# SergioAlvarezB/calibration-normalizing-flows

Measured on AMD Instinct MI355X. Metric: logit-vectors/sec forward+log-det (6-layer RealNVP, D=10), higher is better.
Workload: dtype f32; 1 GPU; cfg2: 6-layer RealNVP coupling, D=10, hidden_size=[5, 5], 1048576 vectors per GPU; global_batch=1048576, parallelism=dp1, weights=N(0,0.1) synthetic

## Files before the change

calibration-normalizing-flows_amd/csrc/cnf_sgpr.hip:

```cpp
#include <hip/hip_runtime.h>

#include <mutex>
#include <type_traits>
#include <unordered_map>

#include "cnf_internal.h"
#include "cnf_valu_common.h"
#include "cnf_valu_io.h"
#include "cnf_sgpr_common.h"

#ifdef CNF_SGPR_TRACE
__device__ unsigned long long cnf_trace[16384 * 8];
__device__ unsigned long long cnf_trace_clk[16384 * 2];
#define CNF_TRC(slot)                                                                   \
  do {                                                                                  \
    if (lane == 0 && gw < 16384) cnf_trace_clk[gw * 2 + (slot)] = __builtin_amdgcn_s_memtime(); \
  } while (0)
#define CNF_TR(slot)                                                                   \
  do {                                                                                 \
    if (lane == 0 && gw < 16384) cnf_trace[gw * 8 + (slot)] = __builtin_amdgcn_s_memrealtime(); \
  } while (0)
#else
#define CNF_TR(slot) \
  do {               \
  } while (0)
#define CNF_TRC(slot) \
  do {                \
  } while (0)
#endif

namespace cnf {
namespace {

using namespace valu;

constexpr int kWaves = 4;

template <bool ALL, bool PERM>
constexpr int pairs_per_lane() { return 1; }
template <int MODE, bool ALL, bool PERM>
constexpr int waves_per_simd() { return PERM ? 4 : 6; }

enum Mode { kFwd = 0, kInv = 1, kLoss = 2, kPredict = 3 };



template <int D, int H1, int H2, int P>
struct Act {
  f2 c[P][D - D / 2];
  f2 h1[P][H1 > 0 ? H1 : 1];
  f2 h2[P][H2 > 0 ? H2 : 1];
  f2 t[P][D / 2];
};

template <int NIN, int NOUT, int S, bool RELU, int P, int NC, class X, class E, class F>
__device__ __forceinline__ void slin(const SW<NC>& w, X&& x, E&& emit, F&& before) {
  sready();
  before();
  f2 a[NOUT][P];
#pragma unroll
  for (int o = 0; o < NOUT; ++o)
#pragma unroll
    for (int q = 0; q < P; ++q) {
      if constexpr (RELU && NIN == 1) a[o][q] = fma_wb_clamp(w.pair(o * S), x(q, 0));
      else a[o][q] = fma_wb(w.pair(o * S), x(q, 0));
    }
#pragma unroll
  for (int k = 1; k < NIN; ++k)
#pragma unroll
    for (int o = 0; o < NOUT; ++o)
#pragma unroll
      for (int q = 0; q < P; ++q) {
        if (RELU && k == NIN - 1) a[o][q] = fma_ws_clamp(w, o * S + 1 + k, x(q, k), a[o][q]);
        else a[o][q] = fma_ws(w, o * S + 1 + k, x(q, k), a[o][q]);
      }
#pragma unroll
  for (int o = 0; o < NOUT; ++o) emit(o, a[o]);
}

template <class S, int NETS, int IDX>
__device__ __forceinline__ constexpr int lin_at() {
  return ((NETS == 2 && IDX < S::NL) ? S::NF : 0) + S::off(IDX % S::NL);
}

template <class S, int NETS, int P, int IDX, int PAR, bool NEXT, class AC, class U>
__device__ __forceinline__ void run_seq(AC& ac, SW<S::NC>& A, SW<S::NC>& Bf, const float* wl,
                                        const float* wn, U&& upd) {
  constexpr int NL = S::NL, N = NETS * NL;
  if constexpr (IDX < N) {
    constexpr int i = IDX % NL;
    constexpr bool tnet = IDX < NL, last = i == NL - 1;
    constexpr bool odd = ((IDX + PAR) & 1) != 0;
    SW<S::NC>& cur = odd ? Bf : A;
    SW<S::NC>& nxt = odd ? A : Bf;
    auto x = [&](int q, int k) -> f2 {
      if constexpr (i == 0) return ac.c[q][k];
      else if constexpr (i == 1) return ac.h1[q][k];
      else return ac.h2[q][k];
    };
    auto emit = [&](int o, const f2* a) {
#pragma unroll
      for (int q = 0; q < P; ++q) {
        if constexpr (!last) {
          if constexpr (i == 0) ac.h1[q][o] = a[q];
          else ac.h2[q][o] = a[q];
        } else if constexpr (tnet && NETS == 2) {
          ac.t[q][o] = a[q];
        }
      }
      if constexpr (last && (!tnet || NETS == 1)) upd(o, a);
    };
    slin<S::nin(i), S::nout(i), S::stride(i), !last, P>(cur, x, emit, [&]() {
      if constexpr (IDX + 1 < N)
        sissue(nxt, wl + lin_at<S, NETS, IDX + 1>());
      else if constexpr (NEXT)
        sissue(nxt, wn + lin_at<S, NETS, 0>());
    });
    run_seq<S, NETS, P, IDX + 1, PAR, NEXT>(ac, A, Bf, wl, wn, upd);
  }
}

template <int D, int H1, int H2, bool INV, bool O, int NETS, bool PERM, bool NEXT, int P>
__device__ __forceinline__ void sp_step(f2 (&v)[P][D], f2 (&ld)[P], SW<SP<D, H1, H2>::NC>& A,
                                        SW<SP<D, H1, H2>::NC>& Bf, const float* wl,
                                        const float* wn, bool perm,
                                        const int32_t* __restrict__ q) {
  using S = SP<D, H1, H2>;
  constexpr int DT = S::DT, DC = S::DC;
  constexpr bool OC = INV ? !O : O;
  if constexpr (INV && PERM) {
    if (perm) {
#pragma unroll
      for (int p = 0; p < P; ++p) permute<D, O>(v[p], q);
    }
  }
  Act<D, H1, H2, P> ac;
#pragma unroll
  for (int p = 0; p < P; ++p)
#pragma unroll
    for (int k = 0; k < DC; ++k) ac.c[p][k] = v[p][R<D, OC>(DT + k)];
  auto upd = [&](int j, const f2* a) {
#pragma unroll
    for (int p = 0; p < P; ++p) {
      f2& x = v[p][R<D, OC>(j)];
      if constexpr (NETS == 1) {
        x = INV ? x - a[p] : x + a[p];
      } else if constexpr (!INV) {
        x = fmaV(x, exp2T(a[p]), ac.t[p][j]);
        ld[p] += a[p];
      } else {
        x = (x - ac.t[p][j]) * exp2T(-a[p]);
        ld[p] -= a[p];
      }
    }
  };
  run_seq<S, NETS, P, 0, O ? (NETS * S::NL) & 1 : 0, NEXT>(ac, A, Bf, wl, wn, upd);
  if constexpr (!INV && PERM) {
    if (perm) {
#pragma unroll
      for (int p = 0; p < P; ++p) permute<D, O>(v[p], q);
    }
  }
}

__device__ __forceinline__ float max3f(float a, float b, float c) {
  float r;
  asm("v_max3_f32 %0, %1, %2, %3" : "=v"(r) : "v"(a), "v"(b), "v"(c));
  return r;
}
__device__ __forceinline__ float max2f(float a, float b) {
  float r;
  asm("v_max_f32 %0, %1, %2" : "=v"(r) : "v"(a), "v"(b));
  return r;
}
template <int D>
__device__ __forceinline__ f2 pair_max(const f2* v) {
  f2 m;
#pragma unroll
  for (int q = 0; q < 2; ++q) {
    float r = v[0][q];
    int j = 1;
#pragma unroll
    for (; j + 1 < D; j += 2) r = max3f(r, v[j][q], v[j + 1][q]);
    if (j < D) r = max2f(r, v[j][q]);
    m[q] = r;
  }
  return m;
}

template <int D, int GATHER>
__device__ __forceinline__ void pair_loss(const f2* v, f2 ld, uint32_t lab2, int rows, int kind,
                                          float det, float& t0, float& t1, float& t2,
                                          const float* tile) {
  const uint32_t b0 = lab2 & 0xffu, b1 = (lab2 >> 8) & 0xffu;
  const bool ok[2] = {b0 != 0xffu, b1 != 0xffu};
  constexpr float kL2E = 1.4426950408889634f, kLN2 = 0.6931471805599453f;
  float zy[2];
  if constexpr (GATHER == 1) {
    zy[0] = tile[ok[0] ? (int)b0 : 0];
    zy[1] = tile[D + (ok[1] ? (int)b1 : 0)];
  }
  const f2 m = pair_max<D>(v);
  const f2 nm = m * splat(-kL2E, f2{});
  f2 se = exp2T(fmaT(kL2E, v[0], nm));
#pragma unroll
  for (int j = 1; j < D; ++j) se += exp2T(fmaT(kL2E, v[j], nm));
  if constexpr (GATHER == 0) {
    uint32_t za[D], zb[D];
#pragma unroll
    for (int j = 0; j < D; ++j) {
      za[j] = __float_as_uint(v[j].x);
      zb[j] = __float_as_uint(v[j].y);
    }
    zy[0] = __uint_as_float(sel_tree<D>(za, ok[0] ? (int)b0 : 0, 0));
    zy[1] = __uint_as_float(sel_tree<D>(zb, ok[1] ? (int)b1 : 0, 0));
  }
#pragma unroll
  for (int q = 0; q < 2; ++q) {
    if (q >= rows) continue;
    const float lpy = zy[q] - (m[q] + __builtin_amdgcn_logf(se[q]) * kLN2);
    const float l = ld[q];
    float ce, loss;
    if (kind == CNF_LOSS_CAL) {
      ce = -__builtin_amdgcn_logf(__builtin_amdgcn_exp2f(lpy * kL2E) + 1e-7f) * kLN2;
      loss = ce - l;
    } else {
      ce = -lpy;
      loss = ce - det * l;
    }
    if (!ok[q]) ce = loss = __builtin_nanf("");
    t0 += loss;
    t1 += ce;
    t2 += l;
  }
}

template <int D, bool O>
__device__ __forceinline__ void centre(f2* v) {
  f2 s = v[R<D, O>(0)];
#pragma unroll
  for (int j = 1; j < D; ++j) s += v[R<D, O>(j)];
  const f2 mu = s * splat(1.f / D, f2{});
#pragma unroll
  for (int j = 0; j < D; ++j) v[j] -= mu;
}

template <int D>
__device__ __forceinline__ void pair_predict(f2* v, const float* __restrict__ lp) {
  constexpr float kL2E = 1.4426950408889634f, kLN2 = 0.6931471805599453f;
  const f2 m = pair_max<D>(v);
  const f2 nm = m * splat(-kL2E, f2{});
  f2 e[D], se = splat(0.f, f2{});
#pragma unroll
  for (int j = 0; j < D; ++j) {
    e[j] = exp2T(fmaT(kL2E, v[j], nm));
    se += e[j];
  }
  const f2 inv = f2{1.f / se.x, 1.f / se.y};
  f2 a[D];
#pragma unroll
  for (int j = 0; j < D; ++j) {
    const f2 p = e[j] * inv + splat(1e-7f, f2{});
    a[j] = f2{__builtin_amdgcn_logf(p.x), __builtin_amdgcn_logf(p.y)} * splat(kLN2, f2{}) -
           splat(lp[j], f2{});
  }
  const f2 m2 = pair_max<D>(a);
  const f2 nm2 = m2 * splat(-kL2E, f2{});
  f2 s2 = splat(0.f, f2{});
#pragma unroll
  for (int j = 0; j < D; ++j) {
    a[j] = exp2T(fmaT(kL2E, a[j], nm2));
    s2 += a[j];
  }
  const f2 inv2 = f2{1.f / s2.x, 1.f / s2.y};
#pragma unroll
  for (int j = 0; j < D; ++j) v[j] = a[j] * inv2;
}

struct KArgs {
  float* out;
  float* ld;
  float* all;
  const int64_t* y;
  float* part;
  const void *reserved0, *reserved1, *reserved2;
  int L, kind;
  float det;
};

template <int D, int H1, int H2, int NETS, int MODE, bool ALL, bool PERM>
__global__ __launch_bounds__(kWaves * 64, (waves_per_simd<MODE, ALL, PERM>())) void k_sgpr(
    const float* __restrict__ in,
    int64_t B,
    const float* __restrict__ W,
    const int32_t* __restrict__ qtab,
    const int32_t* __restrict__ lflag,
    const float* __restrict__ lpri,
    KArgs a) {
  using S = SP<D, H1, H2>;
  constexpr int P = pairs_per_lane<ALL, PERM>();
  constexpr bool INV = MODE == kInv;
  constexpr int LF = NETS * S::NF;
  constexpr int TR = 128 * P;
  constexpr int TF = TR * D;
  extern __shared__ __attribute__((aligned(16))) float smem[];
  const int lane = threadIdx.x & 63;
  const int wv = __builtin_amdgcn_readfirstlane(threadIdx.x >> 6);
  float* sm = smem + wv * TF;
  const int L = a.L;
  const int nfull = (int)(B / TR), ntiles = (int)((B + TR - 1) / TR);
  const int gw = blockIdx.x * kWaves + wv, nw = gridDim.x * kWaves;
  int left = gw < ntiles ? (ntiles - 1 - gw) / nw + 1 : 0;
  auto layer_of = [&](int i) { return INV ? L - 1 - i : i; };
  auto align_of = [](const void* q) {
    const int m = (int)(reinterpret_cast<uintptr_t>(q) & 15);
    return m == 0 ? 16 : ((m & 7) == 0 ? 8 : 4);
  };
  [[maybe_unused]] const int al = a.out ? align_of(a.out) : 16;
  const int al_ld = a.ld ? align_of(a.ld) : 16;
  const bool y16 = MODE == kLoss && (reinterpret_cast<uintptr_t>(a.y) & 15) == 0;
  float lp[MODE == kPredict ? D : 1];
  if constexpr (MODE == kPredict) {
#pragma unroll
    for (int j = 0; j < D; ++j) lp[j] = lpri[j];
  }
  float lt0 = 0.f, lt1 = 0.f, lt2 = 0.f;

  const bool odd = (L & 1) != 0;
  auto compute = [&](f2 (&v)[P][D], f2 (&ld)[P], int64_t row0, int nr) {
#pragma unroll
    for (int p = 0; p < P; ++p) {
      if constexpr (MODE == kPredict) {
        if (odd) centre<D, true>(v[p]);
        else centre<D, false>(v[p]);
      }
      ld[p] = splat(0.f, f2{});
    }
    auto st_all = [&](int i, auto O_) {
      if constexpr (ALL) {
        constexpr bool O = decltype(O_)::value;
        f2 o[P][D];
#pragma unroll
        for (int p = 0; p < P; ++p)
#pragma unroll
          for (int j = 0; j < D; ++j) o[p][j] = v[p][R<D, O>(j)];
        store_rows<D, P>(a.all + ((int64_t)i * B + row0 + 2 * P * lane) * D, o, nr, 16);
      }
    };
    int i = 0;
    if (odd) {
      const int la = layer_of(0);
      const bool pa = PERM && (lflag[la] & kFlagPerm);
      const float* wa = W + (int64_t)la * LF;
      SW<S::NC> cur, alt;
      if constexpr (((NETS * S::NL) & 1) != 0) sissue(alt, wa + lin_at<S, NETS, 0>());
      else sissue(cur, wa + lin_at<S, NETS, 0>());
      sp_step<D, H1, H2, INV, true, NETS, PERM, false, P>(v, ld, cur, alt, wa, nullptr, pa,
                                                          qtab + la * D);
      st_all(0, std::false_type{});
      i = 1;
    }
    for (; i + 1 < L; i += 2) {
      const int la = layer_of(i), lb = layer_of(i + 1);
      const bool pa = PERM && (lflag[la] & kFlagPerm);
      const bool pb = PERM && (lflag[lb] & kFlagPerm);
      const float* wa = W + (int64_t)la * LF;
      const float* wb = W + (int64_t)lb * LF;
      SW<S::NC> cur, alt;
      sissue(cur, wa + lin_at<S, NETS, 0>());
      sp_step<D, H1, H2, INV, false, NETS, PERM, true, P>(v, ld, cur, alt, wa, wb, pa,
                                                          qtab + la * D);
      st_all(i, std::true_type{});
      sp_step<D, H1, H2, INV, true, NETS, PERM, false, P>(v, ld, cur, alt, wb, nullptr, pb,
                                                          qtab + lb * D);
      st_all(i + 1, std::false_type{});
    }
#pragma unroll
    for (int p = 0; p < P; ++p) {
      if constexpr (NETS == 2) ld[p] = ld[p] * splat(0.69314718055994531f, f2{});
      if constexpr (MODE == kPredict) pair_predict<D>(v[p], lp);
    }
  };
  auto loss = [&](const f2 (&v)[P][D], const f2 (&ld)[P], uint32_t lab, int nr,
                  const float* tile, auto gather) {
#pragma unroll
    for (int p = 0; p < P; ++p) {
      const int r = nr - 2 * p;
      constexpr int G = decltype(gather)::value;
      pair_loss<D, G>(v[p], ld[p], lab >> (16 * p), r < 0 ? 0 : (r > 2 ? 2 : r), a.kind, a.det,
                      lt0, lt1, lt2, tile + 2 * D * p);
    }
  };

  CNF_TR(0);
  CNF_TRC(0);
#ifdef CNF_SGPR_TRACE
  if (lane == 0 && gw < 16384)
    cnf_trace[gw * 8 + 7] = ((unsigned long long)__builtin_amdgcn_s_getreg((31 << 11) | 20) << 32) |
                            __builtin_amdgcn_s_getreg((31 << 11) | 4);
  int ntr = 0;
#endif
  int t = gw;
  if (t < nfull) wave_dma<D, TR>(sm, in + (int64_t)t * TF, lane);
  auto set_prio = [&]() {
    --left;
    if (left >= 3) __builtin_amdgcn_s_setprio(3);
    else if (left == 2) __builtin_amdgcn_s_setprio(2);
    else if (left == 1) __builtin_amdgcn_s_setprio(1);
    else __builtin_amdgcn_s_setprio(0);
  };
  for (; t < nfull; t += nw) {
    set_prio();
    asm volatile("s_waitcnt vmcnt(0)" ::: "memory");
    f2 v[P][D];
    if constexpr (P == 1) {
      if (odd) read_pairs_wait<D, true>(sm, lane, v);
      else read_pairs_wait<D, false>(sm, lane, v);
    } else {
      if (odd) read_pairs<D, P, true>(sm, lane, v);
      else read_pairs<D, P, false>(sm, lane, v);
      asm volatile("s_waitcnt lgkmcnt(0)" ::: "memory");
    }
#ifdef CNF_SGPR_TRACE
    if (ntr < 2) CNF_TR(1 + 2 * ntr);
#endif
    const int64_t row0 = (int64_t)t * TR;
    uint32_t lab = 0;
    if constexpr (MODE == kLoss) lab = load_labels<D, P>(a.y + row0 + 2 * P * lane, 2 * P, y16);
    f2 ld[P];
    compute(v, ld, row0, 2 * P);
    if constexpr (MODE == kLoss) {
      stage_pairs<D, P>(sm, lane, v);
      loss(v, ld, lab, 2 * P, sm + 2 * P * D * lane, std::integral_constant<int, 1>{});
    }
#ifdef CNF_SGPR_TRACE
    if (ntr < 2) CNF_TR(2 + 2 * ntr);
    CNF_TR(5);
    ++ntr;
#endif
    if (a.out) {
      if (MODE != kLoss) stage_pairs<D, P>(sm, lane, v);
      store_tile<TF>(a.out + row0 * D, sm, lane);
    }
    if (a.ld) store_lds<P>(a.ld + row0 + 2 * P * lane, ld, 2 * P, al_ld);
    asm volatile("s_waitcnt lgkmcnt(0)" ::: "memory");
    if (t + nw < nfull) wave_dma<D, TR>(sm, in + (int64_t)(t + nw) * TF, lane);
  }
  if (t == nfull && nfull < ntiles) {
    const int64_t row0 = (int64_t)t * TR;
    const int64_t r = row0 + 2 * P * lane;
    const int64_t left_rows = B - r;
    const int nr = left_rows <= 0 ? 0 : (left_rows >= 2 * P ? 2 * P : (int)left_rows);
    f2 v[P][D];
    auto load_rows = [&](auto O_) {
      constexpr bool O = decltype(O_)::value;
#pragma unroll
      for (int p = 0; p < P; ++p)
#pragma unroll
        for (int k = 0; k < D; ++k) {
          v[p][R<D, O>(k)].x = 2 * p < nr ? in[(r + 2 * p) * D + k] : 0.f;
          v[p][R<D, O>(k)].y = 2 * p + 1 < nr ? in[(r + 2 * p + 1) * D + k] : 0.f;
        }
    };
    if (odd) load_rows(std::true_type{});
    else load_rows(std::false_type{});
    uint32_t lab = 0;
    if constexpr (MODE == kLoss) lab = load_labels<D, P>(a.y + r, nr, false);
    f2 ld[P];
    compute(v, ld, row0, nr);
    if constexpr (MODE == kLoss) loss(v, ld, lab, nr, sm, std::integral_constant<int, 0>{});
    if (a.out) store_rows<D, P>(a.out + r * D, v, nr, 4);
    if (a.ld) store_lds<P>(a.ld + r, ld, nr, 4);
  }
  CNF_TRC(1);
  CNF_TR(6);
  if constexpr (MODE == kLoss) block_sum3<kWaves * 64>(lt0, lt1, lt2, smem, a.part);
}

using KFn = void (*)(const float*, int64_t, const float*, const int32_t*, const int32_t*,
                     const float*, KArgs);

struct KV {
  KFn fn;
  int tr;
};

enum Var { vFwd, vInv, vLoss, vPredict, kNVar };

struct SEntry {
  int D, H1, H2;
  KV fn[2][kNVar];
  KV pfn[2][3];
};

#define CNF_K(D, H1, H2, N, M, A, P) \
  {k_sgpr<D, H1, H2, N, M, A, P>, 128 * pairs_per_lane<A, P>()}
#define CNF_SV(D, H1, H2, N)                                                                  \
  {CNF_K(D, H1, H2, N, kFwd, false, false), CNF_K(D, H1, H2, N, kInv, false, false),           \
   CNF_K(D, H1, H2, N, kLoss, false, false), CNF_K(D, H1, H2, N, kPredict, false, false)}
#define CNF_SP(D, H1, H2, N)                                                                  \
  {CNF_K(D, H1, H2, N, kFwd, false, true), CNF_K(D, H1, H2, N, kInv, false, true),             \
   CNF_K(D, H1, H2, N, kPredict, false, true)}
#define CNF_SGPR(D, H1, H2) \
  {D, H1, H2, {CNF_SV(D, H1, H2, 1), CNF_SV(D, H1, H2, 2)}, {CNF_SP(D, H1, H2, 1), CNF_SP(D, H1, H2, 2)}}

const SEntry kSTable[] = {
#ifdef CNF_SGPR_DEV
    CNF_SGPR(10, 5, 5),
#else
    CNF_SGPR(2, 5, 5), CNF_SGPR(3, 5, 5), CNF_SGPR(4, 5, 5), CNF_SGPR(5, 5, 5),
    CNF_SGPR(6, 5, 5), CNF_SGPR(8, 5, 5), CNF_SGPR(10, 5, 5),
    CNF_SGPR(3, 3, 3), CNF_SGPR(8, 3, 3), CNF_SGPR(10, 3, 3),
    CNF_SGPR(3, 3, 0), CNF_SGPR(3, 0, 0), CNF_SGPR(10, 0, 0),
    CNF_SGPR(10, 5, 0), CNF_SGPR(3, 5, 0),
#endif
};

const SEntry* find(const Shape& s) {
  const int h1 = s.n_lin >= 2 ? s.units[1] : 0, h2 = s.n_lin >= 3 ? s.units[2] : 0;
  for (const SEntry& e : kSTable)
    if (e.D == s.D && e.H1 == h1 && e.H2 == h2) return &e;
  return nullptr;
}

size_t lds_bytes(const Shape& s, const KV& k) {
  return (size_t)kWaves * k.tr * s.D * 4;
}

int resident_blocks(const KV& k, size_t lds) {
  static std::mutex mu;
  static std::unordered_map<const void*, int> cache;
  std::lock_guard<std::mutex> g(mu);
  auto it = cache.find((const void*)k.fn);
  if (it != cache.end()) return it->second;
  int n = 0, dev = 0, cus = 0;
  if (hipOccupancyMaxActiveBlocksPerMultiprocessor(&n, k.fn, kWaves * 64, lds) != hipSuccess ||
      n < 1)
    n = 1;
  constexpr int kGridWps = 6;
  if (n > kGridWps * 4 / kWaves) n = kGridWps * 4 / kWaves;
  if (hipGetDevice(&dev) != hipSuccess ||
      hipDeviceGetAttribute(&cus, hipDeviceAttributeMultiprocessorCount, dev) != hipSuccess ||
      cus < 1)
    cus = 256;
  cache[(const void*)k.fn] = n * cus;
  return n * cus;
}

const KV* pick(const SEntry* e, const Shape& s, int mode, bool all) {
  const int n = s.scale ? 1 : 0;
  if (all) return nullptr;
  if (s.any_perm) {
    if (mode == kLoss) return nullptr;
    return &e->pfn[n][mode == kInv ? 1 : (mode == kPredict ? 2 : 0)];
  }
  return &e->fn[n][mode];
}

int64_t grid_for(const KV& k, const Shape& s, int64_t B) {
  const int64_t ntiles = (B + k.tr - 1) / k.tr;
  const int64_t want = (ntiles + kWaves - 1) / kWaves;
  int64_t cap = resident_blocks(k, lds_bytes(s, k));
  static const int cus = []() {
    int dev = 0, c = 0;
    if (hipGetDevice(&dev) != hipSuccess ||
        hipDeviceGetAttribute(&c, hipDeviceAttributeMultiprocessorCount, dev) != hipSuccess ||
        c < 1)
      c = 256;
    return c;
  }();
  const int64_t simds = (int64_t)cus * 4, wmax = cap / cus;
  if (ntiles % simds == 0) {
    const int64_t T = ntiles / simds;
    if (T <= 24 && T % wmax != 0)
      for (int64_t w = wmax - 1; w >= 4; --w)
        if (T % w == 0) {
          cap = w * cus;
          break;
        }
  }
  return want < cap ? want : cap;
}

bool io_ok(const void* p, int64_t align) {
  return p == nullptr || (reinterpret_cast<uintptr_t>(p) % align) == 0;
}

}

bool sgpr_enabled(const Shape& s) {
  return s.sp_ok && !s.strict && s.shift && !s.alt_mask && !s.s_tanh && find(s) &&
         !(s.options & CNF_OPT_NO_SGPR);
}

int64_t sgpr_blocks(const Shape& s, int64_t B) {
  const SEntry* e = find(s);
  const KV* k = e ? pick(e, s, kLoss, false) : nullptr;
  return k ? grid_for(*k, s, B) : 0;
}

int sgpr_run(const Shape& s, const void* prepared, const float* in, float* out, float* ld,
             float* all, int64_t B, bool inverse, hipStream_t st, const int64_t* y,
             float* loss_ws, int kind, float det, float* loss_terms, const float* log_priors) {
  const SEntry* e = find(s);
  if (!e || !sgpr_enabled(s)) return CNF_ERR_UNSUPPORTED;
  if (B == 0) return CNF_OK;
  if (B / 128 > 0x7fffffffLL) return CNF_ERR_UNSUPPORTED;
  if (!io_ok(in, 16) || !io_ok(out, 16) || !io_ok(all, 16) || !io_ok(ld, 4))
    return CNF_ERR_UNSUPPORTED;
  const int mode = log_priors ? kPredict : (loss_ws ? kLoss : (inverse ? kInv : kFwd));
  const KV* k = pick(e, s, mode, all != nullptr);
  if (!k) return CNF_ERR_UNSUPPORTED;
  const char* base = static_cast<const char*>(prepared);
  const int32_t* fwd_q = reinterpret_cast<const int32_t*>(base);
  const int32_t* inv_q = fwd_q + s.L * s.D;
  const int32_t* flags = inv_q + s.L * s.D;
  const float* W = reinterpret_cast<const float*>(base + idx_bytes(s)) + s.sp_region;
  KArgs a{};
  a.out = out;
  a.ld = ld;
  a.all = all;
  a.y = y;
  a.part = loss_ws ? loss_ws + 4 : nullptr;
  a.L = s.L;
  a.kind = kind;
  a.det = det;
  const int64_t nblk = grid_for(*k, s, B);
  hipLaunchKernelGGL(k->fn, dim3((unsigned)nblk), dim3(kWaves * 64), lds_bytes(s, *k), st, in, B,
                     W, inverse ? inv_q : fwd_q, flags, log_priors, a);
  if (mode == kLoss) reduce_partials(loss_ws + 4, (int)nblk, 4, 0, nullptr, loss_terms, st);
  hipError_t err = hipGetLastError();
  if (err != hipSuccess) {
    set_hip_error(err);
    return CNF_ERR_HIP;
  }
  return CNF_OK;
}

}

#ifdef CNF_SGPR_TRACE
extern "C" int cnf_diag_trace_clk(unsigned long long* host, int n) {
  if (n > 16384 * 2) n = 16384 * 2;
  return hipMemcpyFromSymbol(host, HIP_SYMBOL(cnf_trace_clk), (size_t)n * 8, 0,
                             hipMemcpyDeviceToHost) == hipSuccess ? n : -1;
}
extern "C" int cnf_diag_trace(unsigned long long* host, int n) {
  if (n > 16384 * 8) n = 16384 * 8;
  return hipMemcpyFromSymbol(host, HIP_SYMBOL(cnf_trace), (size_t)n * 8, 0,
                             hipMemcpyDeviceToHost) == hipSuccess ? n : -1;
}
#endif
```

calibration-normalizing-flows_amd/csrc/cnf_sgpr_common.h:

```cpp
#pragma once
#include <hip/hip_runtime.h>

#include <cstdint>

#include "cnf_valu_common.h"

namespace cnf {
namespace valu {

template <int D, int H1, int H2>
struct SP {
  static constexpr int DT = D / 2, DC = D - D / 2;
  static constexpr int NL = H1 == 0 ? 1 : (H2 == 0 ? 2 : 3);
  static constexpr int nin(int i) { return i == 0 ? DC : (i == 1 ? H1 : H2); }
  static constexpr int nout(int i) { return i == NL - 1 ? DT : (i == 0 ? H1 : H2); }
  static constexpr int stride(int i) { return (nin(i) + 2) & ~1; }
  static constexpr int fl(int i) { return pad16(nout(i) * stride(i)); }
  static constexpr int off(int i) { return i == 0 ? 0 : off(i - 1) + fl(i - 1); }
  static constexpr int NF = off(NL);
  static constexpr int mx(int i) { return i == NL ? 0 : (fl(i) > mx(i + 1) ? fl(i) : mx(i + 1)); }
  static constexpr int NC = mx(0) / 16;
  static_assert(NC >= 1 && NC <= 2, "Linear block exceeds the 32-float SGPR buffer");
};

template <int NC>
struct SW {
  v16f c[NC];
  __device__ __forceinline__ float operator[](int i) const { return c[i >> 4][i & 15]; }
  __device__ __forceinline__ f2 pair(int i) const {
    return f2{c[i >> 4][i & 15], c[i >> 4][(i & 15) + 1]};
  }
};

__device__ __forceinline__ f2 fma_wb(f2 wb, f2 x) {
  f2 a;
  asm("v_pk_fma_f32 %0, %1, %2, %1 op_sel:[0,0,1] op_sel_hi:[0,1,1]" : "=v"(a) : "s"(wb), "v"(x));
  return a;
}
__device__ __forceinline__ f2 fma_wb_clamp(f2 wb, f2 x) {
  f2 a;
  asm("v_pk_fma_f32 %0, %1, %2, %1 op_sel:[0,0,1] op_sel_hi:[0,1,1] clamp"
      : "=v"(a) : "s"(wb), "v"(x));
  return a;
}
__device__ __forceinline__ f2 fma_clamp(float w, f2 x, f2 acc) {
  f2 a;
  asm("v_pk_fma_f32 %0, %1, %2, %3 op_sel_hi:[0,1,1] clamp" : "=v"(a) : "s"(f2{w, w}), "v"(x),
      "v"(acc));
  return a;
}

template <int NC>
__device__ __forceinline__ f2 fma_ws(const SW<NC>& w, int idx, f2 x, f2 acc) {
  const f2 p = w.pair(idx & ~1);
  f2 a;
  if (idx & 1)
    asm("v_pk_fma_f32 %0, %1, %2, %3 op_sel:[1,0,0] op_sel_hi:[1,1,1]"
        : "=v"(a) : "s"(p), "v"(x), "v"(acc));
  else
    asm("v_pk_fma_f32 %0, %1, %2, %3 op_sel_hi:[0,1,1]" : "=v"(a) : "s"(p), "v"(x), "v"(acc));
  return a;
}
template <int NC>
__device__ __forceinline__ f2 fma_ws_clamp(const SW<NC>& w, int idx, f2 x, f2 acc) {
  const f2 p = w.pair(idx & ~1);
  f2 a;
  if (idx & 1)
    asm("v_pk_fma_f32 %0, %1, %2, %3 op_sel:[1,0,0] op_sel_hi:[1,1,1] clamp"
        : "=v"(a) : "s"(p), "v"(x), "v"(acc));
  else
    asm("v_pk_fma_f32 %0, %1, %2, %3 op_sel_hi:[0,1,1] clamp"
        : "=v"(a) : "s"(p), "v"(x), "v"(acc));
  return a;
}

template <int NC>
__device__ __forceinline__ f2 mul_ws(const SW<NC>& w, int idx, f2 x) {
  const f2 p = w.pair(idx & ~1);
  f2 a;
  if (idx & 1)
    asm("v_pk_mul_f32 %0, %1, %2 op_sel:[1,0] op_sel_hi:[1,1]" : "=v"(a) : "s"(p), "v"(x));
  else
    asm("v_pk_mul_f32 %0, %1, %2 op_sel_hi:[0,1]" : "=v"(a) : "s"(p), "v"(x));
  return a;
}

__device__ __forceinline__ void sready() {
  __builtin_amdgcn_sched_barrier(0);
  __builtin_amdgcn_s_waitcnt(0xC07F);
  __builtin_amdgcn_sched_barrier(0);
}
template <int NC>
__device__ __forceinline__ void sissue(SW<NC>& r, const float* p) {
  const v16f* q = reinterpret_cast<const v16f*>(__builtin_assume_aligned(p, 64));
#pragma unroll
  for (int i = 0; i < NC; ++i) r.c[i] = q[i];
  __builtin_amdgcn_sched_barrier(0);
}

constexpr int kDmaAux = 2;
template <int D, int TR>
__device__ __forceinline__ void wave_dma(float* sm, const float* __restrict__ src, int lane) {
  constexpr int N4 = TR * D / 4, NI = (N4 + 63) / 64;
#pragma unroll
  for (int i = 0; i < NI; ++i) {
    if (N4 % 64 == 0 || i * 64 + lane < N4)
      __builtin_amdgcn_global_load_lds(src + (i * 64 + lane) * 4,
                                       (__attribute__((address_space(3))) void*)(sm + i * 256), 16,
                                       0, kDmaAux);
  }
}

template <int D, int P, bool REV = false>
__device__ __forceinline__ void read_pairs(const float* sm, int lane, f2 (&v)[P][D]) {
  const float* b = sm + 2 * P * D * lane;
#pragma unroll
  for (int p = 0; p < P; ++p)
#pragma unroll
    for (int k = 0; k < D; ++k)
      v[p][REV ? D - 1 - k : k] = f2{b[2 * p * D + k], b[(2 * p + 1) * D + k]};
}

#define CNF_RP_L(k) "ds_read2_b32 %" #k ", %[b] offset0:" #k " offset1:%[d]+" #k "\n\t"
#define CNF_RP_O(k) "=&v"(o[k])
#define CNF_RPL2 CNF_RP_L(0) CNF_RP_L(1)
#define CNF_RPL3 CNF_RPL2 CNF_RP_L(2)
#define CNF_RPL4 CNF_RPL3 CNF_RP_L(3)
#define CNF_RPL5 CNF_RPL4 CNF_RP_L(4)
#define CNF_RPL6 CNF_RPL5 CNF_RP_L(5)
#define CNF_RPL7 CNF_RPL6 CNF_RP_L(6)
#define CNF_RPL8 CNF_RPL7 CNF_RP_L(7)
#define CNF_RPL9 CNF_RPL8 CNF_RP_L(8)
#define CNF_RPL10 CNF_RPL9 CNF_RP_L(9)
#define CNF_RPL11 CNF_RPL10 CNF_RP_L(10)
#define CNF_RPL12 CNF_RPL11 CNF_RP_L(11)
#define CNF_RPL13 CNF_RPL12 CNF_RP_L(12)
#define CNF_RPL14 CNF_RPL13 CNF_RP_L(13)
#define CNF_RPL15 CNF_RPL14 CNF_RP_L(14)
#define CNF_RPL16 CNF_RPL15 CNF_RP_L(15)
#define CNF_RPO2 CNF_RP_O(0), CNF_RP_O(1)
#define CNF_RPO3 CNF_RPO2, CNF_RP_O(2)
#define CNF_RPO4 CNF_RPO3, CNF_RP_O(3)
#define CNF_RPO5 CNF_RPO4, CNF_RP_O(4)
#define CNF_RPO6 CNF_RPO5, CNF_RP_O(5)
#define CNF_RPO7 CNF_RPO6, CNF_RP_O(6)
#define CNF_RPO8 CNF_RPO7, CNF_RP_O(7)
#define CNF_RPO9 CNF_RPO8, CNF_RP_O(8)
#define CNF_RPO10 CNF_RPO9, CNF_RP_O(9)
#define CNF_RPO11 CNF_RPO10, CNF_RP_O(10)
#define CNF_RPO12 CNF_RPO11, CNF_RP_O(11)
#define CNF_RPO13 CNF_RPO12, CNF_RP_O(12)
#define CNF_RPO14 CNF_RPO13, CNF_RP_O(13)
#define CNF_RPO15 CNF_RPO14, CNF_RP_O(14)
#define CNF_RPO16 CNF_RPO15, CNF_RP_O(15)
template <int D>
__device__ __forceinline__ void ds_read2_pairs(uint32_t base, f2* o);
#define CNF_RPW(D)                                                                   \
  template <>                                                                        \
  __device__ __forceinline__ void ds_read2_pairs<D>(uint32_t base, f2 * o) {         \
    asm volatile(CNF_RPL##D "s_waitcnt lgkmcnt(0)"                                   \
                 : CNF_RPO##D                                                        \
                 : [b] "v"(base), [d] "i"(D)                                         \
                 : "memory");                                                        \
  }
CNF_RPW(2) CNF_RPW(3) CNF_RPW(4) CNF_RPW(5) CNF_RPW(6) CNF_RPW(7) CNF_RPW(8) CNF_RPW(9)
CNF_RPW(10) CNF_RPW(11) CNF_RPW(12) CNF_RPW(13) CNF_RPW(14) CNF_RPW(15) CNF_RPW(16)
#undef CNF_RPW

template <int D, bool REV = false>
__device__ __forceinline__ void read_pairs_wait(const float* sm, int lane, f2 (&v)[1][D]) {
  static_assert(D >= 2 && D <= 16, "ds_read2_pairs is specialised for 2 <= D <= 16");
  typedef __attribute__((address_space(3))) const float lds_f;
  const uint32_t base = (uint32_t)(uintptr_t)(lds_f*)(sm + 2 * D * lane);
  f2 o[D];
  ds_read2_pairs<D>(base, o);
#pragma unroll
  for (int k = 0; k < D; ++k) v[0][REV ? D - 1 - k : k] = o[k];
}

template <int D, int P>
__device__ __forceinline__ void stage_pairs(float* sm, int lane, const f2 (&v)[P][D]) {
  static_assert(2 * P * D <= 256, "ds_write2_b32 dword offsets are 8-bit");
  typedef __attribute__((address_space(3))) float lds_f;
  const uint32_t base = (uint32_t)(uintptr_t)(lds_f*)(sm + 2 * P * D * lane);
#pragma unroll
  for (int p = 0; p < P; ++p)
#pragma unroll
    for (int k = 0; k < D; ++k)
      asm volatile("ds_write2_b32 %0, %1, %2 offset0:%3 offset1:%4"
                   :
                   : "v"(base), "v"(v[p][k].x), "v"(v[p][k].y), "i"(2 * p * D + k),
                     "i"((2 * p + 1) * D + k)
                   : "memory");
}
template <int TF>
__device__ __forceinline__ void store_tile(float* __restrict__ dst, const float* sm, int lane) {
  constexpr int N4 = TF / 4, NI = (N4 + 63) / 64;
  static_assert(TF % 4 == 0, "tile must be whole float4s");
  float4 q[NI];
#pragma unroll
  for (int i = 0; i < NI; ++i)
    if (N4 % 64 == 0 || i * 64 + lane < N4)
      q[i] = *reinterpret_cast<const float4*>(sm + (i * 64 + lane) * 4);
#pragma unroll
  for (int i = 0; i < NI; ++i)
    if (N4 % 64 == 0 || i * 64 + lane < N4) {
      using v4 = __attribute__((ext_vector_type(4))) float;
      __builtin_nontemporal_store(v4{q[i].x, q[i].y, q[i].z, q[i].w},
                                  reinterpret_cast<v4*>(dst) + i * 64 + lane);
    }
}

template <int D, int P>
__device__ __forceinline__ void store_rows(float* __restrict__ dst, const f2 (&v)[P][D], int rows,
                                           int al) {
  constexpr int NF = 2 * P * D;
  float r[NF];
#pragma unroll
  for (int p = 0; p < P; ++p)
#pragma unroll
    for (int k = 0; k < D; ++k) {
      r[2 * p * D + k] = v[p][k].x;
      r[(2 * p + 1) * D + k] = v[p][k].y;
    }
  if (rows == 2 * P && NF % 4 == 0 && al >= 16) {
#pragma unroll
    for (int q = 0; q < NF / 4; ++q)
      reinterpret_cast<float4*>(dst)[q] = float4{r[4 * q], r[4 * q + 1], r[4 * q + 2], r[4 * q + 3]};
  } else if (rows == 2 * P && NF % 2 == 0 && al >= 8) {
#pragma unroll
    for (int q = 0; q < NF / 2; ++q) reinterpret_cast<float2*>(dst)[q] = float2{r[2 * q], r[2 * q + 1]};
  } else {
#pragma unroll
    for (int k = 0; k < NF; ++k)
      if (k < rows * D) dst[k] = r[k];
  }
}

template <int P>
__device__ __forceinline__ void store_lds(float* __restrict__ dst, const f2 (&ld)[P], int rows,
                                          int al) {
  if (P == 2 && rows == 4 && al >= 16) {
    *reinterpret_cast<float4*>(dst) = float4{ld[0].x, ld[0].y, ld[P - 1].x, ld[P - 1].y};
  } else if (rows == 2 * P && al >= 8) {
#pragma unroll
    for (int p = 0; p < P; ++p) {
      reinterpret_cast<float2*>(dst)[p] = float2{ld[p].x, ld[p].y};
    }
  } else {
#pragma unroll
    for (int p = 0; p < P; ++p) {
      if (2 * p < rows) dst[2 * p] = ld[p].x;
      if (2 * p + 1 < rows) dst[2 * p + 1] = ld[p].y;
    }
  }
}

template <int D>
__device__ __forceinline__ void unflip(f2* v) {
#pragma unroll
  for (int k = 0; k < D / 2; ++k) {
    const f2 a = v[k];
    v[k] = v[D - 1 - k];
    v[D - 1 - k] = a;
  }
}

template <int D, int P>
__device__ __forceinline__ uint32_t load_labels(const int64_t* __restrict__ y, int rows,
                                                bool al16) {
  uint32_t packed = 0;
  const int32_t* y32 = reinterpret_cast<const int32_t*>(y);
#pragma unroll
  for (int p = 0; p < P; ++p) {
    int lo0 = 0, hi0 = 0, lo1 = 0, hi1 = 0;
    if (rows == 2 * P && al16) {
      const int4 q = reinterpret_cast<const int4*>(y32)[p];
      lo0 = q.x, hi0 = q.y, lo1 = q.z, hi1 = q.w;
    } else {
      if (2 * p < rows) lo0 = y32[4 * p], hi0 = y32[4 * p + 1];
      if (2 * p + 1 < rows) lo1 = y32[4 * p + 2], hi1 = y32[4 * p + 3];
    }
    const uint32_t b0 = hi0 == 0 && (unsigned)lo0 < (unsigned)D ? (uint32_t)lo0 : 0xffu;
    const uint32_t b1 = hi1 == 0 && (unsigned)lo1 < (unsigned)D ? (uint32_t)lo1 : 0xffu;
    packed |= (b0 | (b1 << 8)) << (16 * p);
  }
  return packed;
}

}
}
```

Before: 38.11 billion logit-vectors/sec.

## Cut SGPR pressure by re-reading kernargs and hand-scheduling 5x5 linear layer

Adds a single inline-asm block for the 5x5 hidden linear layer (P==1) so the packed FMAs are emitted back to back with scalar weight operands. Kernel arguments (out, ld, y, in, B, kind, det, L parity) are re-read from the kernarg segment at each use instead of being held live across the loop, which is meant to free scalar registers. Label decoding is moved after compute, and the weight pointer is advanced by a stride instead of being recomputed each iteration. The cost is extra scalar loads and more fragile inline asm.

```diff
diff --git a/calibration-normalizing-flows_amd/csrc/cnf_sgpr.hip b/calibration-normalizing-flows_amd/csrc/cnf_sgpr.hip
--- a/calibration-normalizing-flows_amd/csrc/cnf_sgpr.hip
+++ b/calibration-normalizing-flows_amd/csrc/cnf_sgpr.hip
@@ -57,6 +57,14 @@
 __device__ __forceinline__ void slin(const SW<NC>& w, X&& x, E&& emit, F&& before) {
   sready();
   before();
+  if constexpr (NIN == 5 && NOUT == 5 && S == 6 && NC == 2 && P == 1) {
+    const f2 x5[5] = {x(0, 0), x(0, 1), x(0, 2), x(0, 3), x(0, 4)};
+    f2 a5[5];
+    lin5x5<RELU>(w, x5, a5);
+#pragma unroll
+    for (int o = 0; o < NOUT; ++o) emit(o, &a5[o]);
+    return;
+  }
   f2 a[NOUT][P];
 #pragma unroll
   for (int o = 0; o < NOUT; ++o)
@@ -189,16 +197,14 @@
 }
 
 template <int D, int GATHER>
-__device__ __forceinline__ void pair_loss(const f2* v, f2 ld, uint32_t lab2, int rows, int kind,
-                                          float det, float& t0, float& t1, float& t2,
-                                          const float* tile) {
-  const uint32_t b0 = lab2 & 0xffu, b1 = (lab2 >> 8) & 0xffu;
-  const bool ok[2] = {b0 != 0xffu, b1 != 0xffu};
+__device__ __forceinline__ void pair_loss(const f2* v, f2 ld, const int (&idx)[2],
+                                          const bool (&ok)[2], int rows, int kind, float det,
+                                          float& t0, float& t1, float& t2, const float* tile) {
   constexpr float kL2E = 1.4426950408889634f, kLN2 = 0.6931471805599453f;
   float zy[2];
   if constexpr (GATHER == 1) {
-    zy[0] = tile[ok[0] ? (int)b0 : 0];
-    zy[1] = tile[D + (ok[1] ? (int)b1 : 0)];
+    zy[0] = tile[idx[0]];
+    zy[1] = tile[D + idx[1]];
   }
   const f2 m = pair_max<D>(v);
   const f2 nm = m * splat(-kL2E, f2{});
@@ -212,13 +218,14 @@
       za[j] = __float_as_uint(v[j].x);
       zb[j] = __float_as_uint(v[j].y);
     }
-    zy[0] = __uint_as_float(sel_tree<D>(za, ok[0] ? (int)b0 : 0, 0));
-    zy[1] = __uint_as_float(sel_tree<D>(zb, ok[1] ? (int)b1 : 0, 0));
+    zy[0] = __uint_as_float(sel_tree<D>(za, idx[0], 0));
+    zy[1] = __uint_as_float(sel_tree<D>(zb, idx[1], 0));
   }
 #pragma unroll
   for (int q = 0; q < 2; ++q) {
     if (q >= rows) continue;
-    const float lpy = zy[q] - (m[q] + __builtin_amdgcn_logf(se[q]) * kLN2);
+    const float zq = ok[q] ? zy[q] : __builtin_nanf("");
+    const float lpy = zq - (m[q] + __builtin_amdgcn_logf(se[q]) * kLN2);
     const float l = ld[q];
     float ce, loss;
     if (kind == CNF_LOSS_CAL) {
@@ -228,7 +235,6 @@
       ce = -lpy;
       loss = ce - det * l;
     }
-    if (!ok[q]) ce = loss = __builtin_nanf("");
     t0 += loss;
     t1 += ce;
     t2 += l;
@@ -283,10 +289,27 @@
   float* all;
   const int64_t* y;
   float* part;
-  const void *reserved0, *reserved1, *reserved2;
   int L, kind;
   float det;
 };
+
+struct KBlock {
+  const float* in;
+  int64_t B;
+  const float *W;
+  const int32_t *qtab, *lflag;
+  const float* lpri;
+  KArgs a;
+};
+typedef const __attribute__((address_space(4))) KBlock* KBlockPtr;
+typedef const __attribute__((address_space(4))) KArgs* KArgsPtr;
+
+__device__ __forceinline__ KBlockPtr fresh_block() {
+  KBlockPtr p = (KBlockPtr)__builtin_amdgcn_kernarg_segment_ptr();
+  asm volatile("" : "+s"(p));
+  return p;
+}
+__device__ __forceinline__ KArgsPtr fresh_args() { return &fresh_block()->a; }
 
 template <int D, int H1, int H2, int NETS, int MODE, bool ALL, bool PERM>
 __global__ __launch_bounds__(kWaves * 64, (waves_per_simd<MODE, ALL, PERM>())) void k_sgpr(
@@ -316,9 +339,6 @@
     const int m = (int)(reinterpret_cast<uintptr_t>(q) & 15);
     return m == 0 ? 16 : ((m & 7) == 0 ? 8 : 4);
   };
-  [[maybe_unused]] const int al = a.out ? align_of(a.out) : 16;
-  const int al_ld = a.ld ? align_of(a.ld) : 16;
-  const bool y16 = MODE == kLoss && (reinterpret_cast<uintptr_t>(a.y) & 15) == 0;
   float lp[MODE == kPredict ? D : 1];
   if constexpr (MODE == kPredict) {
 #pragma unroll
@@ -326,12 +346,16 @@
   }
   float lt0 = 0.f, lt1 = 0.f, lt2 = 0.f;
 
-  const bool odd = (L & 1) != 0;
+  auto is_odd = [&]() {
+    int l = L;
+    asm volatile("" : "+s"(l));
+    return (l & 1) != 0;
+  };
   auto compute = [&](f2 (&v)[P][D], f2 (&ld)[P], int64_t row0, int nr) {
 #pragma unroll
     for (int p = 0; p < P; ++p) {
       if constexpr (MODE == kPredict) {
-        if (odd) centre<D, true>(v[p]);
+        if (is_odd()) centre<D, true>(v[p]);
         else centre<D, false>(v[p]);
       }
       ld[p] = splat(0.f, f2{});
@@ -348,7 +372,7 @@
       }
     };
     int i = 0;
-    if (odd) {
+    if (is_odd()) {
       const int la = layer_of(0);
       const bool pa = PERM && (lflag[la] & kFlagPerm);
       const float* wa = W + (int64_t)la * LF;
@@ -360,12 +384,13 @@
       st_all(0, std::false_type{});
       i = 1;
     }
-    for (; i + 1 < L; i += 2) {
+    constexpr int LS = INV ? -LF : LF;
+    const float* wa = W + (int64_t)layer_of(i) * LF;
+    for (; i + 1 < L; i += 2, wa += 2 * LS) {
       const int la = layer_of(i), lb = layer_of(i + 1);
       const bool pa = PERM && (lflag[la] & kFlagPerm);
       const bool pb = PERM && (lflag[lb] & kFlagPerm);
-      const float* wa = W + (int64_t)la * LF;
-      const float* wb = W + (int64_t)lb * LF;
+      const float* wb = wa + LS;
       SW<S::NC> cur, alt;
       sissue(cur, wa + lin_at<S, NETS, 0>());
       sp_step<D, H1, H2, INV, false, NETS, PERM, true, P>(v, ld, cur, alt, wa, wb, pa,
@@ -381,14 +406,27 @@
       if constexpr (MODE == kPredict) pair_predict<D>(v[p], lp);
     }
   };
-  auto loss = [&](const f2 (&v)[P][D], const f2 (&ld)[P], uint32_t lab, int nr,
-                  const float* tile, auto gather) {
+  auto loss = [&](const f2 (&v)[P][D], const f2 (&ld)[P], const auto& labels, int nr,
+                  const float* tile, int kind, float det, auto gather) {
 #pragma unroll
     for (int p = 0; p < P; ++p) {
       const int r = nr - 2 * p;
       constexpr int G = decltype(gather)::value;
-      pair_loss<D, G>(v[p], ld[p], lab >> (16 * p), r < 0 ? 0 : (r > 2 ? 2 : r), a.kind, a.det,
-                      lt0, lt1, lt2, tile + 2 * D * p);
+      bool ok[2];
+      int idx[2];
+#pragma unroll
+      for (int q = 0; q < 2; ++q) {
+        if constexpr (G == 1) {
+          ok[q] = (uint64_t)labels[2 * p + q] < (uint64_t)D;
+          idx[q] = ok[q] ? (int)labels[2 * p + q] : 0;
+        } else {
+          const uint32_t b = (labels >> (16 * p + 8 * q)) & 0xffu;
+          ok[q] = b != 0xffu;
+          idx[q] = ok[q] ? (int)b : 0;
+        }
+      }
+      pair_loss<D, G>(v[p], ld[p], idx, ok, r < 0 ? 0 : (r > 2 ? 2 : r), kind, det, lt0, lt1, lt2,
+                      tile + 2 * D * p);
     }
   };
 
@@ -414,10 +452,10 @@
     asm volatile("s_waitcnt vmcnt(0)" ::: "memory");
     f2 v[P][D];
     if constexpr (P == 1) {
-      if (odd) read_pairs_wait<D, true>(sm, lane, v);
+      if (is_odd()) read_pairs_wait<D, true>(sm, lane, v);
       else read_pairs_wait<D, false>(sm, lane, v);
     } else {
-      if (odd) read_pairs<D, P, true>(sm, lane, v);
+      if (is_odd()) read_pairs<D, P, true>(sm, lane, v);
       else read_pairs<D, P, false>(sm, lane, v);
       asm volatile("s_waitcnt lgkmcnt(0)" ::: "memory");
     }
@@ -425,31 +463,47 @@
     if (ntr < 2) CNF_TR(1 + 2 * ntr);
 #endif
     const int64_t row0 = (int64_t)t * TR;
-    uint32_t lab = 0;
-    if constexpr (MODE == kLoss) lab = load_labels<D, P>(a.y + row0 + 2 * P * lane, 2 * P, y16);
+    int64_t lab[2 * P] = {};
+    if constexpr (MODE == kLoss) {
+      const int64_t* y = fresh_args()->y;
+      load_labels_raw<P>(y + row0 + 2 * P * lane, (reinterpret_cast<uintptr_t>(y) & 15) == 0,
+                         lab);
+    }
     f2 ld[P];
     compute(v, ld, row0, 2 * P);
+    const KArgsPtr ka = fresh_args();
+    float* const out = ka->out;
+    float* const ldo = ka->ld;
     if constexpr (MODE == kLoss) {
+      int kind = ka->kind;
+      float det = ka->det;
+      asm volatile("" : "+s"(kind), "+s"(det));
       stage_pairs<D, P>(sm, lane, v);
-      loss(v, ld, lab, 2 * P, sm + 2 * P * D * lane, std::integral_constant<int, 1>{});
+      loss(v, ld, lab, 2 * P, sm + 2 * P * D * lane, kind, det, std::integral_constant<int, 1>{});
     }
 #ifdef CNF_SGPR_TRACE
     if (ntr < 2) CNF_TR(2 + 2 * ntr);
     CNF_TR(5);
     ++ntr;
 #endif
-    if (a.out) {
+    if (out) {
       if (MODE != kLoss) stage_pairs<D, P>(sm, lane, v);
-      store_tile<TF>(a.out + row0 * D, sm, lane);
-    }
-    if (a.ld) store_lds<P>(a.ld + row0 + 2 * P * lane, ld, 2 * P, al_ld);
+      store_tile<TF>(out + row0 * D, sm, lane);
+    }
+    if (ldo) store_lds<P>(ldo + row0 + 2 * P * lane, ld, 2 * P, align_of(ldo));
     asm volatile("s_waitcnt lgkmcnt(0)" ::: "memory");
-    if (t + nw < nfull) wave_dma<D, TR>(sm, in + (int64_t)(t + nw) * TF, lane);
-  }
-  if (t == nfull && nfull < ntiles) {
+    if (t + nw < nfull) {
+      typedef __attribute__((address_space(3))) float lds_f;
+      uint32_t sa = (uint32_t)(uintptr_t)(lds_f*)sm;
+      asm volatile("" : "+s"(sa));
+      wave_dma<D, TR>((lds_f*)(uintptr_t)sa, fresh_block()->in + (int64_t)(t + nw) * TF, lane);
+    }
+  }
+  if (t == nfull && fresh_block()->B % TR != 0) {
+    const float* __restrict__ in = fresh_block()->in;
     const int64_t row0 = (int64_t)t * TR;
     const int64_t r = row0 + 2 * P * lane;
-    const int64_t left_rows = B - r;
+    const int64_t left_rows = fresh_block()->B - r;
     const int nr = left_rows <= 0 ? 0 : (left_rows >= 2 * P ? 2 * P : (int)left_rows);
     f2 v[P][D];
     auto load_rows = [&](auto O_) {
@@ -462,19 +516,23 @@
           v[p][R<D, O>(k)].y = 2 * p + 1 < nr ? in[(r + 2 * p + 1) * D + k] : 0.f;
         }
     };
-    if (odd) load_rows(std::true_type{});
+    if (is_odd()) load_rows(std::true_type{});
     else load_rows(std::false_type{});
     uint32_t lab = 0;
-    if constexpr (MODE == kLoss) lab = load_labels<D, P>(a.y + r, nr, false);
+    if constexpr (MODE == kLoss) lab = load_labels<D, P>(fresh_args()->y + r, nr, false);
     f2 ld[P];
     compute(v, ld, row0, nr);
-    if constexpr (MODE == kLoss) loss(v, ld, lab, nr, sm, std::integral_constant<int, 0>{});
-    if (a.out) store_rows<D, P>(a.out + r * D, v, nr, 4);
-    if (a.ld) store_lds<P>(a.ld + r, ld, nr, 4);
+    const KArgsPtr ka = fresh_args();
+    float* const out = ka->out;
+    float* const ldo = ka->ld;
+    if constexpr (MODE == kLoss)
+      loss(v, ld, lab, nr, sm, ka->kind, ka->det, std::integral_constant<int, 0>{});
+    if (out) store_rows<D, P>(out + r * D, v, nr, 4);
+    if (ldo) store_lds<P>(ldo + r, ld, nr, 4);
   }
   CNF_TRC(1);
   CNF_TR(6);
-  if constexpr (MODE == kLoss) block_sum3<kWaves * 64>(lt0, lt1, lt2, smem, a.part);
+  if constexpr (MODE == kLoss) block_sum3<kWaves * 64>(lt0, lt1, lt2, smem, fresh_args()->part);
 }
 
 using KFn = void (*)(const float*, int64_t, const float*, const int32_t*, const int32_t*,
diff --git a/calibration-normalizing-flows_amd/csrc/cnf_sgpr_common.h b/calibration-normalizing-flows_amd/csrc/cnf_sgpr_common.h
--- a/calibration-normalizing-flows_amd/csrc/cnf_sgpr_common.h
+++ b/calibration-normalizing-flows_amd/csrc/cnf_sgpr_common.h
@@ -74,6 +74,38 @@
   return a;
 }
 
+#define CNF_L5_0(o) \
+  "v_pk_fma_f32 %[a" #o "], %[p" #o "0], %[x0], %[p" #o "0] op_sel:[0,0,1] op_sel_hi:[0,1,1]\n\t"
+#define CNF_L5_E(o, k, j, C) \
+  "v_pk_fma_f32 %[a" #o "], %[p" #o #j "], %[x" #k "], %[a" #o "] op_sel_hi:[0,1,1]" C "\n\t"
+#define CNF_L5_O(o, k, j, C)                                                                  \
+  "v_pk_fma_f32 %[a" #o "], %[p" #o #j "], %[x" #k "], %[a" #o "] op_sel:[1,0,0] op_sel_hi:[1,1,1]" \
+  C "\n\t"
+#define CNF_L5_ALL(M, ...) \
+  M(0, ##__VA_ARGS__) M(1, ##__VA_ARGS__) M(2, ##__VA_ARGS__) M(3, ##__VA_ARGS__) M(4, ##__VA_ARGS__)
+#define CNF_L5_TEXT(C)                                                                  \
+  CNF_L5_ALL(CNF_L5_0) CNF_L5_ALL(CNF_L5_E, 1, 1, "") CNF_L5_ALL(CNF_L5_O, 2, 1, "")     \
+  CNF_L5_ALL(CNF_L5_E, 3, 2, "") CNF_L5_ALL(CNF_L5_O, 4, 2, C)
+#define CNF_L5_P(o) \
+  [p##o##0] "s"(w.pair(6 * o)), [p##o##1] "s"(w.pair(6 * o + 2)), [p##o##2] "s"(w.pair(6 * o + 4))
+#define CNF_L5_ASM(C)                                                                          \
+  asm(CNF_L5_TEXT(C)                                                                           \
+      : [a0] "=&v"(a[0]), [a1] "=&v"(a[1]), [a2] "=&v"(a[2]), [a3] "=&v"(a[3]), [a4] "=&v"(a[4]) \
+      : [x0] "v"(x[0]), [x1] "v"(x[1]), [x2] "v"(x[2]), [x3] "v"(x[3]), [x4] "v"(x[4]),         \
+        CNF_L5_P(0), CNF_L5_P(1), CNF_L5_P(2), CNF_L5_P(3), CNF_L5_P(4))
+template <bool RELU>
+__device__ __forceinline__ void lin5x5(const SW<2>& w, const f2 (&x)[5], f2 (&a)[5]) {
+  if constexpr (RELU) CNF_L5_ASM(" clamp");
+  else CNF_L5_ASM("");
+}
+#undef CNF_L5_ASM
+#undef CNF_L5_P
+#undef CNF_L5_TEXT
+#undef CNF_L5_ALL
+#undef CNF_L5_O
+#undef CNF_L5_E
+#undef CNF_L5_0
+
 template <int NC>
 __device__ __forceinline__ f2 mul_ws(const SW<NC>& w, int idx, f2 x) {
   const f2 p = w.pair(idx & ~1);
@@ -100,7 +132,8 @@
 
 constexpr int kDmaAux = 2;
 template <int D, int TR>
-__device__ __forceinline__ void wave_dma(float* sm, const float* __restrict__ src, int lane) {
+__device__ __forceinline__ void wave_dma(__attribute__((address_space(3))) float* sm,
+                                         const float* __restrict__ src, int lane) {
   constexpr int N4 = TR * D / 4, NI = (N4 + 63) / 64;
 #pragma unroll
   for (int i = 0; i < NI; ++i) {
@@ -109,6 +142,10 @@
                                        (__attribute__((address_space(3))) void*)(sm + i * 256), 16,
                                        0, kDmaAux);
   }
+}
+template <int D, int TR>
+__device__ __forceinline__ void wave_dma(float* sm, const float* __restrict__ src, int lane) {
+  wave_dma<D, TR>((__attribute__((address_space(3))) float*)sm, src, lane);
 }
 
 template <int D, int P, bool REV = false>
@@ -288,5 +325,19 @@
   return packed;
 }
 
-}
-}
+template <int P>
+__device__ __forceinline__ void load_labels_raw(const int64_t* __restrict__ y, bool al16,
+                                                int64_t (&o)[2 * P]) {
+#pragma unroll
+  for (int p = 0; p < P; ++p) {
+    if (al16) {
+      const longlong2 q = reinterpret_cast<const longlong2*>(y)[p];
+      o[2 * p] = q.x, o[2 * p + 1] = q.y;
+    } else {
+      o[2 * p] = y[2 * p], o[2 * p + 1] = y[2 * p + 1];
+    }
+  }
+}
+
+}
+}
```

New measurement: 38.82 billion logit-vectors/sec (median of 6 runs). +1.9%, better.
